# stjude-rust-labs/ngs

Measured on AMD Instinct MI355X. Metric: BAM records/sec (whole node), all qc facets, 150 bp reads, higher is better.
Workload: dtype u8/u32 integer (u64 accumulators)

## Files before the change

ngs_amd/csrc/cov_scan.hip:

```cpp
#include <hip/hip_runtime.h>

#include "kernels.h"

namespace ngsq {

typedef unsigned long long u64;

constexpr uint32_t CS_THREADS = 256;
constexpr uint32_t CS_PER_THREAD = COV_CHUNK / CS_THREADS;

__device__ __forceinline__ u64 cs_wave_sum64(u64 v) {
#pragma unroll
    for (int o = 32; o > 0; o >>= 1) v += __shfl_down(v, o, 64);
    return v;
}

__global__ __launch_bounds__(COV_SUPER) void k_cov_super_sums(const uint32_t *chunk_sums, uint64_t n_chunks,
                                                             uint32_t *super_sums) {
    __shared__ uint32_t s_w[COV_SUPER / 64];
    const uint64_t i = (uint64_t)blockIdx.x * COV_SUPER + threadIdx.x;
    uint32_t v = i < n_chunks ? chunk_sums[i] : 0u;
#pragma unroll
    for (int o = 32; o > 0; o >>= 1) v += __shfl_down(v, o, 64);
    if ((threadIdx.x & 63) == 0) s_w[threadIdx.x >> 6] = v;
    __syncthreads();
    if (threadIdx.x == 0) {
        uint32_t t = 0;
        for (uint32_t w = 0; w < COV_SUPER / 64; w++) t += s_w[w];
        super_sums[blockIdx.x] = t;
    }
}

constexpr uint32_t CS_STEP = 64 * CS_PER_THREAD;

template <bool RESET, bool SKIP>
__global__ __launch_bounds__(CS_THREADS) void k_cov_scan(CovScanArgs a) {
    extern __shared__ uint32_t s_hist[];
    const uint32_t nb = a.cov_cap + 2;
    const uint32_t tid = threadIdx.x, lane = tid & 63, wave = tid >> 6;
    for (uint32_t i = tid; i < (CS_THREADS / 64) * nb; i += CS_THREADS) s_hist[i] = 0;
    __syncthreads();
    uint32_t *const my_hist = s_hist + wave * nb;

    const uint64_t n_units = (uint64_t)gridDim.x * (CS_THREADS / 64);
    const uint64_t unit = (uint64_t)blockIdx.x * (CS_THREADS / 64) + wave;
    const uint64_t n_range = a.c_end - a.c_begin;
    const uint64_t per = (n_range + n_units - 1) / n_units;
    const uint64_t c_lo = a.c_begin + (per * unit < n_range ? per * unit : n_range);
    const uint64_t c_hi = c_lo + per < a.c_end ? c_lo + per : a.c_end;
    if (c_lo >= c_hi) return;

    uint32_t carry = 0;
    {
        uint32_t part = 0;
        const uint64_t s0 = (a.c_begin + COV_SUPER - 1) / COV_SUPER, s1 = c_lo / COV_SUPER;
        if (s0 < s1) {
            for (uint64_t i = a.c_begin + lane; i < s0 * COV_SUPER; i += 64) part += a.chunk_sums[i];
            for (uint64_t i = s0 + lane; i < s1; i += 64) part += a.super_sums[i];
            for (uint64_t i = s1 * COV_SUPER + lane; i < c_lo; i += 64) part += a.chunk_sums[i];
        } else {
            for (uint64_t i = a.c_begin + lane; i < c_lo; i += 64) part += a.chunk_sums[i];
        }
        if (a.carry_words && ((a.carry_mask >> lane) & 1)) part += a.carry_words[2 * lane];
#pragma unroll
        for (int o = 32; o > 0; o >>= 1) part += __shfl_xor(part, o, 64);
        carry = a.carry_in + part;
    }

    uint32_t ref = 0;
    {
        uint32_t lo = 0, hi = a.n_refs;
        while (hi - lo > 1) {
            const uint32_t mid = (lo + hi) >> 1;
            if (a.ref_first_chunk[mid] <= c_lo) lo = mid; else hi = mid;
        }
        ref = lo;
    }
    bool dirty = false;
    uint64_t L = 0, ref_e0 = 0, ref_e1 = 0;
    u64 *bins = a.bin_totals;
    auto load_ref = [&](uint32_t r) {
        L = a.ref_len[r];
        ref_e0 = (uint64_t)a.ref_first_chunk[r] * COV_CHUNK;
        ref_e1 = (uint64_t)a.ref_first_chunk[r + 1] * COV_CHUNK;
        bins = a.bin_totals + a.bin_off[r];
    };

    uint32_t zeros = 0;
    auto flush_hist = [&](uint32_t r) {
        u64 *dst = a.hist + (u64)r * nb;
        {
            u64 z = zeros;
#pragma unroll
            for (int o = 32; o > 0; o >>= 1) z += __shfl_xor(z, o, 64);
            if (lane == 0 && z) atomicAdd(&dst[0], z);
            zeros = 0;
        }
        for (uint32_t i = lane; i < nb; i += 64) {
            const uint32_t v = my_hist[i];
            if (v) {
                atomicAdd(&dst[i], (u64)v);
                my_hist[i] = 0;
            }
        }
    };
    auto load_step = [&](uint64_t e0, uint4 (&v)[CS_PER_THREAD / 4]) {
        const uint4 *src = reinterpret_cast<const uint4 *>(a.depth + e0 + (uint64_t)lane * CS_PER_THREAD);
#pragma unroll
        for (uint32_t r = 0; r < CS_PER_THREAD / 4; r++) v[r] = src[r];
    };
    auto next_live = [&](uint64_t c) -> uint64_t {
        while (c < c_hi) {
            while (ref + 1 < a.n_refs && c >= a.ref_first_chunk[ref + 1]) {
                if (dirty) flush_hist(ref);
                dirty = false;
                ref += 1;
            }
            if (a.seen[ref] != 0) {
                if (SKIP && a.chunk_flags[c]) {
                    carry += a.chunk_sums[c];
                    c += 1;
                    continue;
                }
                load_ref(ref);
                return c;
            }
            const uint64_t ref_end = a.ref_first_chunk[ref + 1];
            c = ref_end < c_hi ? ref_end : c_hi;
        }
        return c_hi;
    };

    uint64_t c = next_live(c_lo);
    uint64_t e = c * (uint64_t)COV_CHUNK;
    uint4 cur[CS_PER_THREAD / 4];
    if (c < c_hi) load_step(e, cur);
    while (c < c_hi) {
        const uint64_t i0 = e - ref_e0 + (uint64_t)lane * CS_PER_THREAD;
        if (RESET) {
            uint4 *dstz = reinterpret_cast<uint4 *>(a.depth + e + (uint64_t)lane * CS_PER_THREAD);
#pragma unroll
            for (uint32_t r = 0; r < CS_PER_THREAD / 4; r++) dstz[r] = make_uint4(0, 0, 0, 0);
        }
        const uint64_t en = e + CS_STEP;
        bool same_ref = en < c_hi * (uint64_t)COV_CHUNK && en < ref_e1;
        if (SKIP && same_ref && en % COV_CHUNK == 0 && a.chunk_flags[en / COV_CHUNK]) same_ref = false;
        uint4 nxt[CS_PER_THREAD / 4];
        load_step(same_ref ? en : e, nxt);

        uint32_t d[CS_PER_THREAD];
#pragma unroll
        for (uint32_t r = 0; r < CS_PER_THREAD / 4; r++)
            d[4 * r + 0] = cur[r].x, d[4 * r + 1] = cur[r].y, d[4 * r + 2] = cur[r].z, d[4 * r + 3] = cur[r].w;
        uint32_t tsum = 0;
#pragma unroll
        for (uint32_t t = 0; t < CS_PER_THREAD; t++) tsum += d[t];
        uint32_t inc = tsum;
#pragma unroll
        for (int o = 1; o < 64; o <<= 1) {
            const uint32_t t = __shfl_up(inc, o, 64);
            if ((int)lane >= o) inc += t;
        }
        uint32_t run = carry + inc - tsum;
        carry += __shfl(inc, 63, 64);

        const uint32_t nvalid = i0 > L ? 0u : (L - i0 + 1 < CS_PER_THREAD ? (uint32_t)(L - i0 + 1) : CS_PER_THREAD);
        uint32_t q = 0, rem = 0;
        if (i0 >= 1) {
            q = (uint32_t)((i0 - 1) / a.bin_size);
            rem = (uint32_t)((i0 - 1) - (uint64_t)q * a.bin_size);
        }
        u64 bin_sum = 0;
        bool split = false;
#pragma unroll
        for (uint32_t t = 0; t < CS_PER_THREAD; t++) {
            run += d[t];
            if (t < nvalid) {
                const uint32_t depth = run;
                zeros += depth == 0;
                if (depth) atomicAdd(&my_hist[depth <= a.cov_cap ? depth : a.cov_cap + 1], 1u);
                if (i0 + t != 0) {
                    bin_sum += depth;
                    rem += 1;
                    if (rem == a.bin_size) {
                        if (bin_sum) atomicAdd(&bins[(u64)q + 1], bin_sum);
                        bin_sum = 0;
                        rem = 0;
                        q += 1;
                        split = true;
                    }
                }
            }
        }
        const uint32_t q0 = __shfl(q, 0, 64);
        if (__all(!split && q == q0)) {
            const u64 sum = cs_wave_sum64(bin_sum);
            if (lane == 0 && sum) atomicAdd(&bins[(u64)q0 + 1], sum);
        } else if (bin_sum) {
            atomicAdd(&bins[(u64)q + 1], bin_sum);
        }
        dirty = true;
        if (same_ref) {
#pragma unroll
            for (uint32_t r = 0; r < CS_PER_THREAD / 4; r++) cur[r] = nxt[r];
            e = en;
            c = e / COV_CHUNK;
        } else {
            c = next_live((en + COV_CHUNK - 1) / COV_CHUNK);
            e = c * (uint64_t)COV_CHUNK;
            if (c < c_hi) load_step(e, cur);
        }
    }
    if (dirty) flush_hist(ref);
}

hipError_t launch_cov_scan(const LaunchInfo &li, const CovScanArgs &a, hipStream_t s) {
    if (!a.n_chunks) return hipSuccess;
    const size_t lds = (size_t)(CS_THREADS / 64) * (a.cov_cap + 2) * sizeof(uint32_t);
    static bool attr = false;
    if (!attr) {
        const void *fns[4] = {reinterpret_cast<const void *>(k_cov_scan<true, false>), reinterpret_cast<const void *>(k_cov_scan<false, false>),
                              reinterpret_cast<const void *>(k_cov_scan<true, true>), reinterpret_cast<const void *>(k_cov_scan<false, true>)};
        for (const void *f : fns) {
            hipError_t e = hipFuncSetAttribute(f, hipFuncAttributeMaxDynamicSharedMemorySize, 160 * 1024 - 64);
            if (e != hipSuccess) return e;
        }
        attr = true;
    }
    const uint32_t n_super = (uint32_t)((a.n_chunks + COV_SUPER - 1) / COV_SUPER);
    hipLaunchKernelGGL(k_cov_super_sums, dim3(n_super), dim3(COV_SUPER), 0, s, a.chunk_sums, a.n_chunks, a.super_sums);
    if (a.c_end <= a.c_begin) return hipSuccess;
    uint64_t g = (a.c_end - a.c_begin + CS_THREADS / 64 - 1) / (CS_THREADS / 64);
    const uint64_t cap = (uint64_t)li.n_cu * 4;
    if (g > cap) g = cap;
    if (a.reset && a.chunk_flags)
        hipLaunchKernelGGL((k_cov_scan<true, true>), dim3((uint32_t)g), dim3(CS_THREADS), lds, s, a);
    else if (a.reset)
        hipLaunchKernelGGL((k_cov_scan<true, false>), dim3((uint32_t)g), dim3(CS_THREADS), lds, s, a);
    else if (a.chunk_flags)
        hipLaunchKernelGGL((k_cov_scan<false, true>), dim3((uint32_t)g), dim3(CS_THREADS), lds, s, a);
    else
        hipLaunchKernelGGL((k_cov_scan<false, false>), dim3((uint32_t)g), dim3(CS_THREADS), lds, s, a);
    return hipGetLastError();
}

}
```

ngs_amd/csrc/fields_kernel.hip:

```cpp
#include <hip/hip_runtime.h>

#include "kernels.h"

namespace ngsq {

typedef unsigned long long u64;

constexpr uint32_t FT_THREADS = 256;
constexpr uint32_t FT_PER_THREAD = 4;
constexpr uint32_t FT_TILE = FT_THREADS * FT_PER_THREAD;
constexpr uint32_t FT_WINDOW = 2048;
constexpr uint32_t FT_NSLOT = 16 + 3 + 18 + 1 + 1;

__device__ __forceinline__ uint32_t ft_wave_sum(uint32_t v) {
#pragma unroll
    for (int o = 32; o > 0; o >>= 1) v += __shfl_down(v, o, 64);
    return v;
}

__device__ __forceinline__ void ft_chunk_add(uint32_t *chunk_sums, bool active, uint32_t chunk, uint32_t val) {
    const unsigned long long m = __ballot(active);
    if (!m) return;
    const int leader = __ffsll((long long)m) - 1;
    const uint32_t c0 = __shfl(chunk, leader, 64);
    const bool same = active && chunk == c0;
    const uint32_t s = ft_wave_sum(same ? val : 0u);
    if ((threadIdx.x & 63) == 0 && s) atomicAdd(&chunk_sums[c0], s);
    if (active && !same) atomicAdd(&chunk_sums[chunk], val);
}

struct FieldsArgs {
    uint32_t do_general, do_tlen, do_cov;
};

struct FtRaw {
    uint2 flag, ncig;
    uint32_t mapq;
    int4 ref, mate, tlen, pos;
    uint4 cig;
    int32_t prev_ref, prev_pos;
    uint32_t co0;
    uint64_t co_base;
};

__device__ __forceinline__ uint32_t ft_count(bool c) { return (uint32_t)__popcll(__ballot(c)); }

__device__ __forceinline__ uint32_t slot_counter(uint32_t slot) {
    return slot < 16    ? C_GENERAL + slot
           : slot == 16 ? C_ERR + E_MISSING_REF
           : slot == 17 ? C_TLEN_PROCESSED
           : slot == 18 ? C_TLEN_IGNORED
           : slot < 28  ? C_CIGAR1 + (slot - 19)
           : slot < 37  ? C_CIGAR2 + (slot - 28)
           : slot == 37 ? C_ERR + E_BAD_CIGAR
                        : C_COV_UNSORTED;
}

template <bool CIG_OFF, bool STREAM>
__global__ __launch_bounds__(FT_THREADS, 4) void k_fields(DeviceState st, DeviceBatch b, FieldsArgs a) {
    NGSQ_FOREGROUND_WAVE();
    extern __shared__ uint32_t s_dyn[];
    uint32_t *const s_tlen = s_dyn;
    uint32_t *const s_win = s_dyn + ((st.tlen_cap + 1 + 3) & ~3u);
    __shared__ u64 s_acc[FT_NSLOT];
    const uint32_t tid = threadIdx.x, lane = tid & 63;
    for (uint32_t i = tid; i <= st.tlen_cap; i += FT_THREADS) s_tlen[i] = 0;
    if (a.do_cov && !STREAM)
        for (uint32_t i = tid; i < (FT_THREADS / 64) * FT_WINDOW; i += FT_THREADS) s_win[i] = 0;
    if (tid < FT_NSLOT) s_acc[tid] = 0;
    __syncthreads();

    uint32_t g[20];
#pragma unroll
    for (int k = 0; k < 20; k++) g[k] = 0;
    int32_t run_ref = -1;
    uint32_t run_end = 0, max_span = 0;
    uint32_t one[9], two[9];
#pragma unroll
    for (int k = 0; k < 9; k++) one[k] = two[k] = 0;
    u64 pk1 = 0, pk2 = 0;
    uint32_t pk_n = 0;
    auto unpack_ops = [&]() {
#pragma unroll
        for (int q = 0; q < 9; q++) {
            one[q] += (uint32_t)(pk1 >> (7 * q)) & 127u;
            two[q] += (uint32_t)(pk2 >> (7 * q)) & 127u;
        }
        pk1 = pk2 = 0;
        pk_n = 0;
    };
    uint32_t bad_op = 0;
    u64 nonsensical = 0;
    int32_t seen_ref = -1;
    uint32_t seen_cnt = 0;
    u64 t_lo = ~0ull, t_hi = 0;

    const uint64_t n_tiles = (b.n + FT_TILE - 1) / FT_TILE;
    const bool cigar_vec = !CIG_OFF && b.cigar_stride == 1;

    auto load_tile = [&](uint64_t tile) -> FtRaw {
        const uint64_t r0 = tile * FT_TILE + (uint64_t)tid * FT_PER_THREAD;
        FtRaw r;
        r.flag = *reinterpret_cast<const uint2 *>(b.flag + r0);
        r.ncig = make_uint2(0, 0);
        r.mapq = 0;
        r.ref = r.mate = r.tlen = r.pos = make_int4(0, 0, 0, 0);
        r.cig = make_uint4(0, 0, 0, 0);
        if (a.do_general || a.do_cov) {
            r.ref = *reinterpret_cast<const int4 *>(b.ref_id + r0);
            r.ncig = *reinterpret_cast<const uint2 *>(b.n_cigar + r0);
            if (cigar_vec) r.cig = *reinterpret_cast<const uint4 *>(b.cigar + r0);
        }
        if (a.do_general) {
            r.mapq = *reinterpret_cast<const uint32_t *>(b.mapq + r0);
            r.mate = *reinterpret_cast<const int4 *>(b.mate_ref_id + r0);
        }
        if (a.do_tlen) r.tlen = *reinterpret_cast<const int4 *>(b.tlen + r0);
        if (a.do_cov) r.pos = *reinterpret_cast<const int4 *>(b.pos + r0);
        r.co0 = 0;
        r.co_base = 0;
        if (CIG_OFF && (a.do_general || a.do_cov)) {
            r.co_base = b.cigar_off[tile * FT_TILE];
            r.co0 = (uint32_t)(b.cigar_off[r0] - r.co_base);
        }
        r.prev_ref = r.prev_pos = 0;
        if (STREAM) {
            const uint64_t w0 = tile * FT_TILE + (uint64_t)__builtin_amdgcn_readfirstlane((int)(tid >> 6)) * 256;
            const uint64_t pi = w0 ? w0 - 1 : 0;
            r.prev_ref = b.ref_id[pi];
            r.prev_pos = b.pos[pi];
        }
        return r;
    };
    auto load_tail = [&](uint64_t tile, uint32_t &nrec) -> FtRaw {
        const uint64_t r0 = tile * FT_TILE + (uint64_t)tid * FT_PER_THREAD;
        uint32_t flag[4] = {0, 0, 0, 0}, ncig[4] = {0, 0, 0, 0}, mapq[4] = {0, 0, 0, 0}, cig[4] = {0, 0, 0, 0};
        int32_t ref[4] = {0, 0, 0, 0}, mate[4] = {0, 0, 0, 0}, tlen[4] = {0, 0, 0, 0}, pos[4] = {0, 0, 0, 0};
        nrec = 0;
        for (uint32_t j = 0; j < FT_PER_THREAD; j++) {
            if (r0 + j >= b.n) break;
            nrec = j + 1;
            flag[j] = b.flag[r0 + j];
            if (a.do_general || a.do_cov) {
                ref[j] = b.ref_id[r0 + j];
                ncig[j] = b.n_cigar[r0 + j];
                if (cigar_vec) cig[j] = b.cigar[r0 + j];
            }
            if (a.do_general) {
                mapq[j] = b.mapq[r0 + j];
                mate[j] = b.mate_ref_id[r0 + j];
            }
            if (a.do_tlen) tlen[j] = b.tlen[r0 + j];
            if (a.do_cov) pos[j] = b.pos[r0 + j];
        }
        FtRaw r;
        r.flag = make_uint2(flag[0] | (flag[1] << 16), flag[2] | (flag[3] << 16));
        r.ncig = make_uint2(ncig[0] | (ncig[1] << 16), ncig[2] | (ncig[3] << 16));
        r.mapq = mapq[0] | (mapq[1] << 8) | (mapq[2] << 16) | (mapq[3] << 24);
        r.ref = make_int4(ref[0], ref[1], ref[2], ref[3]);
        r.mate = make_int4(mate[0], mate[1], mate[2], mate[3]);
        r.tlen = make_int4(tlen[0], tlen[1], tlen[2], tlen[3]);
        r.pos = make_int4(pos[0], pos[1], pos[2], pos[3]);
        r.cig = make_uint4(cig[0], cig[1], cig[2], cig[3]);
        r.co0 = 0;
        r.co_base = 0;
        r.prev_ref = r.prev_pos = 0;
        if (STREAM && nrec) {
            const uint64_t pi = r0 ? r0 - 1 : 0;
            r.prev_ref = b.ref_id[pi];
            r.prev_pos = b.pos[pi];
        }
        return r;
    };

    int32_t meta_ref = -1;
    uint64_t meta_off = NO_DEPTH, meta_L = 0;
    auto process = [&](const FtRaw &raw, uint64_t tile, uint32_t nrec, bool full_tile) {
        const uint64_t r0 = tile * FT_TILE + (uint64_t)tid * FT_PER_THREAD;
        const uint32_t flag[4] = {raw.flag.x & 0xFFFFu, raw.flag.x >> 16, raw.flag.y & 0xFFFFu, raw.flag.y >> 16};
        const uint32_t ncig[4] = {raw.ncig.x & 0xFFFFu, raw.ncig.x >> 16, raw.ncig.y & 0xFFFFu, raw.ncig.y >> 16};
        const int32_t ref[4] = {raw.ref.x, raw.ref.y, raw.ref.z, raw.ref.w};
        const int32_t mate[4] = {raw.mate.x, raw.mate.y, raw.mate.z, raw.mate.w};
        const int32_t tlen[4] = {raw.tlen.x, raw.tlen.y, raw.tlen.z, raw.tlen.w};
        const int32_t pos[4] = {raw.pos.x, raw.pos.y, raw.pos.z, raw.pos.w};
        const uint32_t cig1[4] = {raw.cig.x, raw.cig.y, raw.cig.z, raw.cig.w};

        uint32_t *const win = s_win + (tid >> 6) * FT_WINDOW;
        int32_t win_ref = -1;
        uint32_t win_base = 0;
        uint64_t win_off = NO_DEPTH, win_L = 0;
        if (a.do_cov) {
            const int32_t fr = __builtin_amdgcn_readfirstlane(ref[0]), fp = __builtin_amdgcn_readfirstlane(pos[0]);
            if (fr >= 0 && (uint32_t)fr < st.n_refs && fp >= 0) {
                if (fr != meta_ref) {
                    const uint64_t o = st.ref_depth_off[fr];
                    const uint32_t l = st.ref_len[fr];
                    meta_ref = fr;
                    meta_off = ((uint64_t)(uint32_t)__builtin_amdgcn_readfirstlane((int)(o >> 32)) << 32) |
                               (uint32_t)__builtin_amdgcn_readfirstlane((int)(uint32_t)o);
                    meta_L = (uint32_t)__builtin_amdgcn_readfirstlane((int)l);
                }
                win_off = meta_off;
                win_L = meta_L;
                if (win_off != NO_DEPTH || STREAM) {
                    win_ref = fr;
                    win_base = (uint32_t)fp & ~3u;
                }
            }
        }
        if (a.do_cov) {
            const int32_t fr = __builtin_amdgcn_readfirstlane(ref[0]);
            const bool stale = seen_cnt != 0 && seen_ref != fr;
            const u64 sm = __ballot(stale);
            if (sm) {
                const int32_t rr = __shfl(seen_ref, __ffsll((long long)sm) - 1, 64);
                const bool same = stale && seen_ref == rr;
                const uint32_t sum = ft_wave_sum(same ? seen_cnt : 0u);
                if (lane == 0 && sum) atomicAdd(&st.counters[st.off_seen + rr], (u64)sum);
                if (stale && !same) atomicAdd(&st.counters[st.off_seen + seen_ref], (u64)seen_cnt);
                if (stale) seen_cnt = 0;
            }
            if (STREAM) {
                const bool stale_e = run_end != 0 && run_ref != fr;
                const u64 em = __ballot(stale_e);
                if (em) {
                    const int32_t rr = __shfl(run_ref, __ffsll((long long)em) - 1, 64);
                    const bool same = stale_e && run_ref == rr;
                    uint32_t m = same ? run_end : 0u;
#pragma unroll
                    for (int o = 32; o > 0; o >>= 1) m = max(m, (uint32_t)__shfl_xor(m, o, 64));
                    if (lane == 0 && m) atomicMax(&st.end_acc[rr], m);
                    if (stale_e && !same) atomicMax(&st.end_acc[run_ref], run_end);
                    if (stale_e) run_end = 0;
                }
            }
        }
        uint32_t my_max = 0;
        uint32_t cend[4] = {0, 0, 0, 0};
        if (STREAM) {
            auto key = [](int32_t rf, int32_t ps) -> u64 {
                return rf < 0 ? 0xFFFFFFFF00000000ull : ((u64)(uint32_t)rf << 32) | (uint32_t)(ps + 1);
            };
            u64 kp = key(raw.prev_ref, raw.prev_pos);
            if (full_tile) {
                const int32_t nr = __shfl_up(ref[3], 1, 64), np_ = __shfl_up(pos[3], 1, 64);
                if (lane) kp = key(nr, np_);
            }
#pragma unroll
            for (uint32_t j = 0; j < FT_PER_THREAD; j++) {
                const u64 kj = key(ref[j], pos[j]);
                g[19] += ft_count(j < nrec && kj < kp);
                kp = kj;
            }
        }

        uint64_t coff[FT_PER_THREAD + 1] = {0, 0, 0, 0, 0};
        uint32_t cigf[FT_PER_THREAD] = {0, 0, 0, 0}, cig2[FT_PER_THREAD] = {0, 0, 0, 0}, cig3[FT_PER_THREAD] = {0, 0, 0, 0};
        if (CIG_OFF && (a.do_general || a.do_cov)) {
            const bool saturated = ncig[0] == 0xFFFFu || ncig[1] == 0xFFFFu || ncig[2] == 0xFFFFu || ncig[3] == 0xFFFFu;
            if (full_tile && !saturated) {
                coff[0] = raw.co_base + raw.co0;
#pragma unroll
                for (uint32_t j = 0; j < FT_PER_THREAD; j++) coff[j + 1] = coff[j] + ncig[j];
            } else if (full_tile) {
                ulonglong2 c01, c23;
                __builtin_memcpy(&c01, b.cigar_off + r0, 16);
                __builtin_memcpy(&c23, b.cigar_off + r0 + 2, 16);
                coff[0] = c01.x, coff[1] = c01.y, coff[2] = c23.x, coff[3] = c23.y;
                coff[4] = b.cigar_off[r0 + 4];
            } else {
#pragma unroll
                for (uint32_t j = 0; j <= FT_PER_THREAD; j++)
                    if (j <= nrec && nrec) coff[j] = b.cigar_off[r0 + j];
            }
#pragma unroll
            for (uint32_t j = 0; j < FT_PER_THREAD; j++) {
                const uint64_t nj = j < nrec ? coff[j + 1] - coff[j] : 0;
                if (nj > 0) cigf[j] = b.cigar[coff[j]];
                if (nj > 1) cig2[j] = b.cigar[coff[j] + 1];
                if (nj > 2) cig3[j] = b.cigar[coff[j] + 2];
            }
        }
#pragma unroll
        for (uint32_t j = 0; j < FT_PER_THREAD; j++) {
            const bool live = j < nrec;
            bool fb = false;
            uint32_t fb_c0 = 0, fb_c1 = 0;
            const uint32_t f = flag[j];
            if (a.do_general) {
                const bool prim = live && !(f & 0x900u);
                const bool pair = prim && (f & 0x1u);
                const bool pmap = pair && !(f & 0x4u);
                const bool mm = pmap && !(f & 0x8u);
                const bool noid = mm && (ref[j] < 0 || mate[j] < 0);
                const bool mis = mm && !noid && ref[j] != mate[j];
                const uint32_t mq = (raw.mapq >> (8 * j)) & 0xFFu;
                g[0] += ft_count(live);
                g[1] += ft_count(live && (f & 0x4u));
                g[2] += ft_count(live && (f & 0x400u));
                g[3] += ft_count(prim);
                g[4] += ft_count(live && (f & 0x100u));
                g[5] += ft_count(live && (f & 0x900u) == 0x800u);
                g[6] += ft_count(prim && !(f & 0x4u));
                g[7] += ft_count(prim && (f & 0x400u));
                g[8] += ft_count(pair);
                g[9] += ft_count(pair && (f & 0x40u));
                g[10] += ft_count(pair && (f & 0x80u));
                g[11] += ft_count(pmap && (f & 0x2u));
                g[12] += ft_count(pmap && (f & 0x8u));
                g[13] += ft_count(mm);
                g[14] += ft_count(mis);
                g[15] += ft_count(mis && mq >= 5u);
                g[16] += ft_count(noid);
            }
            if (a.do_tlen) {
                const int32_t t = tlen[j];
                const bool inr = live && t >= 0 && (uint32_t)t <= st.tlen_cap;
                if (inr) atomicAdd(&s_tlen[t], 1u);
                g[17] += ft_count(inr);
                g[18] += ft_count(live && !inr);
            }
            if ((a.do_general || a.do_cov) && live) {
                uint32_t n_ops = ncig[j];
                const uint32_t r1 = (f >> 6) & 1u;
                uint64_t span = 0;
                uint64_t cbase = (r0 + j) * (uint64_t)b.cigar_stride;
                if (CIG_OFF) {
                    cbase = coff[j];
                    if (n_ops == 0xFFFFu) n_ops = (uint32_t)(coff[j + 1] - cbase);
                }
                for (uint32_t k = 0; k < n_ops; k++) {
                    const uint32_t cg = (cigar_vec && k == 0) ? cig1[j]
                                        : (CIG_OFF && k < 3) ? (k == 0 ? cigf[j] : k == 1 ? cig2[j] : cig3[j])
                                                             : b.cigar[cbase + k];
                    const uint32_t op = cg & 0xFu, len = cg >> 4;
                    if (op > 8u) {
                        bad_op += 1;
                        continue;
                    }
                    if ((0x18Du >> op) & 1u) span += len;
                    if (a.do_general) {
                        const u64 inc = 1ull << (7u * op);
                        pk1 += r1 ? inc : 0ull;
                        pk2 += r1 ? 0ull : inc;
                        if (++pk_n == 127u) unpack_ops();
                    }
                }
                if (a.do_cov) {
                    const int32_t rf = ref[j];
                    const int32_t ps = pos[j];
                    auto cover = [&](uint64_t off, uint64_t L, bool in_seq) {
                        const uint64_t s = (uint64_t)ps + 1, e = s + span - 1;
                        if (off == NO_DEPTH || e == 0 || s > L) return;
                        if (rf != seen_ref) {
                            if (seen_cnt) atomicAdd(&st.counters[st.off_seen + seen_ref], (u64)seen_cnt);
                            seen_ref = rf;
                            seen_cnt = 0;
                        }
                        seen_cnt += 1;
                        const uint64_t ec = e < L ? e : L;
                        nonsensical += e - ec;
                        if (s > ec) return;
                        if (STREAM) {
                            cend[j] = (uint32_t)ec + 1;
                            if (rf != run_ref) {
                                if (run_end) atomicMax(&st.end_acc[run_ref], run_end);
                                run_ref = rf;
                                run_end = 0;
                            }
                            run_end = max(run_end, (uint32_t)ec + 1);
                            max_span = max(max_span, (uint32_t)(ec + 1 - s));
                            return;
                        }
                        const uint64_t i0 = s - win_base, i1 = ec + 1 - win_base;
                        if (in_seq && s >= win_base && i1 < FT_WINDOW) {
                            atomicAdd(&win[i0], 1u);
                            atomicAdd(&win[i1], 0xFFFFFFFFu);
                            my_max = max(my_max, (uint32_t)i1);
                        } else {
                            const uint64_t g0 = off + s, g1 = off + ec + 1;
                            atomicAdd(&st.depth[g0], 1u);
                            atomicAdd(&st.depth[g1], 0xFFFFFFFFu);
                            fb = true;
                            t_lo = g0 < t_lo ? g0 : t_lo;
                            t_hi = g1 + 1 > t_hi ? g1 + 1 : t_hi;
                            fb_c0 = (uint32_t)(g0 / COV_CHUNK);
                            fb_c1 = (uint32_t)(g1 / COV_CHUNK);
                        }
                    };
                    if (rf >= 0 && (uint32_t)rf < st.n_refs && ps >= 0) {
                        if (rf == win_ref) {
                            cover(win_off, win_L, true);
                        } else {
                            cover(st.ref_depth_off[rf], st.ref_len[rf], false);
                        }
                    }
                }
            }
            if (a.do_cov && !STREAM) {
                ft_chunk_add(st.chunk_sums, fb, fb_c0, 1u);
                ft_chunk_add(st.chunk_sums, fb, fb_c1, 0xFFFFFFFFu);
            }
        }

        if (STREAM) {
            if (nrec == FT_PER_THREAD) {
                *reinterpret_cast<uint4 *>(st.cov_end + r0) = make_uint4(cend[0], cend[1], cend[2], cend[3]);
            } else {
                for (uint32_t j = 0; j < nrec; j++) st.cov_end[r0 + j] = cend[j];
            }
        }
        if (a.do_cov && !STREAM) {
#pragma unroll
            for (int o = 32; o > 0; o >>= 1) my_max = max(my_max, (uint32_t)__shfl_xor(my_max, o, 64));
            __builtin_amdgcn_fence(__ATOMIC_ACQ_REL, "wavefront");
            __builtin_amdgcn_wave_barrier();
            const uint32_t top = my_max;
            if (win_ref >= 0 && top) {
                const uint64_t goff = win_off + win_base;
                uint32_t *dst = st.depth + goff;
                t_lo = goff < t_lo ? goff : t_lo;
                t_hi = goff + top + 1 > t_hi ? goff + top + 1 : t_hi;
                const uint32_t c0 = (uint32_t)(goff / COV_CHUNK);
                const uint32_t split = (uint32_t)((uint64_t)(c0 + 1) * COV_CHUNK - goff);
                uint32_t sa = 0, sb = 0;
                for (uint32_t ib = 0; ib <= top; ib += 256) {
                    uint32_t v[4];
#pragma unroll
                    for (uint32_t k = 0; k < 4; k++) {
                        const uint32_t i = ib + 64 * k + lane;
                        v[k] = i < FT_WINDOW ? win[i] : 0u;
                    }
#pragma unroll
                    for (uint32_t k = 0; k < 4; k++) {
                        const uint32_t i = ib + 64 * k + lane;
                        if (v[k]) {
                            atomicAdd(&dst[i], v[k]);
                            win[i] = 0;
                            if (i < split) sa += v[k]; else sb += v[k];
                        }
                    }
                }
                sa = ft_wave_sum(sa);
                sb = ft_wave_sum(sb);
                if (lane == 0) {
                    if (sa) atomicAdd(&st.chunk_sums[c0], sa);
                    if (sb) atomicAdd(&st.chunk_sums[c0 + 1], sb);
                }
                __builtin_amdgcn_fence(__ATOMIC_ACQ_REL, "wavefront");
                __builtin_amdgcn_wave_barrier();
            }
        }
    };

    const uint64_t n_full = b.n / FT_TILE;
    uint64_t tile = blockIdx.x;
    if (tile < n_full) {
        FtRaw cur = load_tile(tile);
        while (tile < n_full) {
            const uint64_t nt = tile + gridDim.x;
            const FtRaw nxt = load_tile(nt < n_full ? nt : tile);
            process(cur, tile, FT_PER_THREAD, true);
            cur = nxt;
            tile = nt;
        }
    }
    if (tile == n_full && n_full < n_tiles) {
        uint32_t nrec = 0;
        const FtRaw tail = load_tail(tile, nrec);
        process(tail, tile, nrec, false);
    }

    {
        const u64 act = __ballot(seen_cnt != 0);
        if (act) {
            const int leader = __ffsll((long long)act) - 1;
            const int32_t rr = __shfl(seen_ref, leader, 64);
            const bool same = seen_cnt != 0 && seen_ref == rr;
            const uint32_t sum = ft_wave_sum(same ? seen_cnt : 0u);
            if (lane == 0) atomicAdd(&st.counters[st.off_seen + rr], (u64)sum);
            if (seen_cnt != 0 && !same) atomicAdd(&st.counters[st.off_seen + seen_ref], (u64)seen_cnt);
        }
    }
    if (STREAM) {
        __shared__ int32_t s_end_ref;
        __shared__ uint32_t s_end_max, s_span_max;
        if (tid == 0) {
            s_end_ref = -1;
            s_end_max = 0;
            s_span_max = 0;
        }
        __syncthreads();
        {
            const u64 act = __ballot(run_end != 0);
            const int32_t wr = __shfl(run_ref, act ? __ffsll((long long)act) - 1 : 0, 64);
            if (act && lane == 0) atomicCAS(&s_end_ref, -1, wr);
        }
        __syncthreads();
        const int32_t lead = s_end_ref;
        const bool same = run_end != 0 && run_ref == lead;
        uint32_t m = same ? run_end : 0u;
#pragma unroll
        for (int o = 32; o > 0; o >>= 1) {
            m = max(m, (uint32_t)__shfl_xor(m, o, 64));
            max_span = max(max_span, (uint32_t)__shfl_xor(max_span, o, 64));
        }
        if (lane == 0 && m) atomicMax(&s_end_max, m);
        if (lane == 0 && max_span) atomicMax(&s_span_max, max_span);
        if (run_end != 0 && !same) atomicMax(&st.end_acc[run_ref], run_end);
        __syncthreads();
        if (tid == 0) {
            if (s_end_max) atomicMax(&st.end_acc[lead], s_end_max);
            if (s_span_max) atomicMax(st.batch_span, s_span_max);
        }
    }
    if (a.do_cov && !STREAM) {
#pragma unroll
        for (int o = 32; o > 0; o >>= 1) {
            const u64 l2 = __shfl_xor(t_lo, o, 64), h2 = __shfl_xor(t_hi, o, 64);
            t_lo = l2 < t_lo ? l2 : t_lo;
            t_hi = h2 > t_hi ? h2 : t_hi;
        }
        if (lane == 0 && t_hi > 0) {
            atomicMin(&st.touched[0], t_lo);
            atomicMax(&st.touched[1], t_hi);
        }
    }
    {
        u64 ns = nonsensical;
#pragma unroll
        for (int o = 32; o > 0; o >>= 1) ns += __shfl_down(ns, o, 64);
        if (lane == 0 && ns) atomicAdd(&st.counters[C_COV_NONSENSICAL], ns);
    }
    if (lane == 0) {
#pragma unroll
        for (int k = 0; k < 19; k++)
            if (g[k]) atomicAdd(&s_acc[k], (u64)g[k]);
        if (g[19]) atomicAdd(&s_acc[38], (u64)g[19]);
    }
    unpack_ops();
#pragma unroll
    for (int k = 0; k < 9; k++) {
        const uint32_t r1 = ft_wave_sum(one[k]), r2 = ft_wave_sum(two[k]);
        if (lane == 0 && r1) atomicAdd(&s_acc[19 + k], (u64)r1);
        if (lane == 0 && r2) atomicAdd(&s_acc[28 + k], (u64)r2);
    }
    {
        const uint32_t r = ft_wave_sum(bad_op);
        if (lane == 0 && r) atomicAdd(&s_acc[37], (u64)r);
    }
    __syncthreads();
    for (uint32_t i = tid; i <= st.tlen_cap; i += FT_THREADS) {
        const uint32_t v = s_tlen[i];
        if (v) atomicAdd(&st.counters[st.off_tlen + i], (u64)v);
    }
    if (tid < FT_NSLOT) {
        const u64 r = s_acc[tid];
        if (r) atomicAdd(&st.counters[slot_counter(tid)], r);
    }
}

hipError_t launch_fields(const LaunchInfo &li, const DeviceState &st, const DeviceBatch &b, uint32_t rec_facets,
                         int coverage, hipStream_t s) {
    if (!b.n) return hipSuccess;
    FieldsArgs a;
    a.do_general = (rec_facets & NGSQ_FACET_GENERAL) ? 1 : 0;
    a.do_tlen = (rec_facets & NGSQ_FACET_TEMPLATE_LENGTH) ? 1 : 0;
    a.do_cov = coverage ? 1 : 0;
    const bool stream = coverage == 2;
    const size_t lds = (((size_t)st.tlen_cap + 1 + 3) & ~(size_t)3) * 4 + (coverage == 1 ? (FT_THREADS / 64) * FT_WINDOW * 4 : 0);
    static bool attr = false;
    if (!attr) {
        const void *fns[4] = {reinterpret_cast<const void *>(k_fields<false, false>), reinterpret_cast<const void *>(k_fields<true, false>),
                              reinterpret_cast<const void *>(k_fields<false, true>), reinterpret_cast<const void *>(k_fields<true, true>)};
        for (const void *f : fns) {
            hipError_t e = hipFuncSetAttribute(f, hipFuncAttributeMaxDynamicSharedMemorySize, 100 * 1024);
            if (e != hipSuccess) return e;
        }
        attr = true;
    }
    uint64_t g = (b.n + FT_TILE - 1) / FT_TILE;
    const uint64_t cap = (uint64_t)li.n_cu * 4;
    if (g > cap) g = cap;
    if (b.cigar_off && stream)
        hipLaunchKernelGGL((k_fields<true, true>), dim3((uint32_t)g), dim3(FT_THREADS), lds, s, st, b, a);
    else if (b.cigar_off)
        hipLaunchKernelGGL((k_fields<true, false>), dim3((uint32_t)g), dim3(FT_THREADS), lds, s, st, b, a);
    else if (stream)
        hipLaunchKernelGGL((k_fields<false, true>), dim3((uint32_t)g), dim3(FT_THREADS), lds, s, st, b, a);
    else
        hipLaunchKernelGGL((k_fields<false, false>), dim3((uint32_t)g), dim3(FT_THREADS), lds, s, st, b, a);
    return hipGetLastError();
}

}
```

Before: 18.46 billion.

## Wave-parallel skip of flagged coverage chunks and contiguous tile ranges per block

In the coverage scan, skipped chunks were walked one at a time by each wave. They are now examined 64 at a time: a ballot finds the first unflagged chunk and a shuffle reduction adds the skipped chunk sums into the carry. In the fields kernel, each block now handles a contiguous range of tiles instead of striding by grid size, which should improve locality for the per-reference and per-chunk accumulation. The tail tile is assigned to the last block. Contiguous ranges can leave the load imbalanced, and the tail block's work may overlap with its full tiles.

```diff
diff --git a/ngs_amd/csrc/cov_scan.hip b/ngs_amd/csrc/cov_scan.hip
--- a/ngs_amd/csrc/cov_scan.hip
+++ b/ngs_amd/csrc/cov_scan.hip
@@ -117,10 +117,24 @@
                 ref += 1;
             }
             if (a.seen[ref] != 0) {
-                if (SKIP && a.chunk_flags[c]) {
-                    carry += a.chunk_sums[c];
-                    c += 1;
-                    continue;
+                if (SKIP) {
+                    const uint64_t ref_end = a.ref_first_chunk[ref + 1];
+                    const uint64_t lim = ref_end < c_hi ? ref_end : c_hi;
+                    uint32_t k = 64;
+                    while (k == 64 && c < lim) {
+                        const bool in = c + lane < lim;
+                        const uint64_t ci = in ? c + lane : lim - 1;
+                        const uint32_t flag = a.chunk_flags[ci];
+                        const uint32_t sum = a.chunk_sums[ci];
+                        const u64 stop = ~__ballot(in && flag != 0);
+                        k = stop ? (uint32_t)__ffsll((long long)stop) - 1 : 64u;
+                        uint32_t part = lane < k ? sum : 0u;
+#pragma unroll
+                        for (int o = 32; o > 0; o >>= 1) part += __shfl_xor(part, o, 64);
+                        carry += part;
+                        c += k;
+                    }
+                    if (c >= lim) continue;
                 }
                 load_ref(ref);
                 return c;
diff --git a/ngs_amd/csrc/fields_kernel.hip b/ngs_amd/csrc/fields_kernel.hip
--- a/ngs_amd/csrc/fields_kernel.hip
+++ b/ngs_amd/csrc/fields_kernel.hip
@@ -454,21 +454,23 @@
     };
 
     const uint64_t n_full = b.n / FT_TILE;
-    uint64_t tile = blockIdx.x;
-    if (tile < n_full) {
+    const uint64_t per = (n_full + gridDim.x - 1) / gridDim.x;
+    uint64_t tile = per * blockIdx.x < n_full ? per * blockIdx.x : n_full;
+    const uint64_t tile_end = tile + per < n_full ? tile + per : n_full;
+    if (tile < tile_end) {
         FtRaw cur = load_tile(tile);
-        while (tile < n_full) {
-            const uint64_t nt = tile + gridDim.x;
-            const FtRaw nxt = load_tile(nt < n_full ? nt : tile);
+        while (tile < tile_end) {
+            const uint64_t nt = tile + 1;
+            const FtRaw nxt = load_tile(nt < tile_end ? nt : tile);
             process(cur, tile, FT_PER_THREAD, true);
             cur = nxt;
             tile = nt;
         }
     }
-    if (tile == n_full && n_full < n_tiles) {
+    if (blockIdx.x == gridDim.x - 1 && n_full < n_tiles) {
         uint32_t nrec = 0;
-        const FtRaw tail = load_tail(tile, nrec);
-        process(tail, tile, nrec, false);
+        const FtRaw tail = load_tail(n_full, nrec);
+        process(tail, n_full, nrec, false);
     }
 
     {
```

Result: no change. 18.46 billion, median of 2 (-0.0%).
